# amcpherson/remixt

Hardware: AMD Instinct MI355X
Metric: EM iterations/sec (50k seg x 165 states) (higher is better)
Workload: dtype f64

## Files before the change

### include/remixt_amd.h

```cpp
#ifndef REMIXT_AMD_H
#define REMIXT_AMD_H

#include <stdint.h>

#ifdef __cplusplus
extern "C" {
#endif

#define RMX_OK 0
#define RMX_EVALUE 1
#define RMX_EASSERT 2
#define RMX_EDEVICE 3
#define RMX_EUNSUPPORTED 4
#define RMX_EARG 5

#define RMX_MAX_CLONES 4

typedef struct rmx_batch rmx_batch;

typedef struct rmx_problem {
    int32_t num_clones;
    int32_t num_segments;
    int32_t num_breakpoints;
    int32_t num_cn_states;
// ... 50 lines not shown
int rmx_info(rmx_batch *b, int32_t what, int64_t *out);
enum rmx_option_id {
    RMX_OPT_FB_KERNEL = 0,
    RMX_OPT_FB_NV,
    RMX_OPT_FB_BREAKEND_CODES,
    RMX_OPT_FUSE_SWEEPS,
    RMX_OPT_TWO_STREAMS,
    RMX_OPT_VITERBI_PLAIN,
    RMX_OPT_SEARCH_MODE,
    RMX_OPT_ELL_DENSE,
    RMX_OPT_STRIP,
    RMX_OPT_CELL_CACHE,
    RMX_OPT_SPARSE_TRIAL,
    RMX_OPT_FB_DEBUG,
    RMX_OPT_PAIRWISE_KERNEL,
    RMX_OPT_PACE_SWEEPS,
    RMX_OPT_FB_WG_BUDGET,
    RMX_OPT_TRIAL_KERNEL,
    RMX_OPT_GRAD_KERNEL,
    RMX_OPT_STREAM_POOL,
    RMX_OPT_VITERBI_CLUSTER,
    RMX_OPT_TRACEBACK,
    RMX_OPT_LT_CLASSES,
    RMX_OPT_COUNT
};
int rmx_set_default_option(int32_t option_id, int32_t value);
int rmx_set_option(rmx_batch *b, int32_t option_id, int32_t value);
int rmx_get_option(rmx_batch *b, int32_t option_id, int32_t *value);

int rmx_set_param(rmx_batch *b, int32_t r, int32_t param_id, double value);
int rmx_get_param(rmx_batch *b, int32_t r, int32_t param_id, double *value);
int rmx_set_transition_model(rmx_batch *b, int32_t model);
int rmx_set_array(rmx_batch *b, int32_t r, int32_t array_id, const void *host_src);
int rmx_get_array(rmx_batch *b, int32_t r, int32_t array_id, void *host_dst);
int rmx_fetch_indicators(rmx_batch *b, int32_t r0, int32_t r1, const double **total, const double **allele);
int rmx_calculate_log_transmat(rmx_batch *b, int32_t r, double *dst);
int rmx_weighted_search(const double *p, int64_t n, const double *u, int32_t k, int64_t *out, int64_t *positive);
int rmx_weighted_sample_round(const double *w, int64_t n, int64_t stride, double norm, const double *u, int32_t k,
                              int64_t *found, int32_t *nfound, int32_t cap, int64_t *positive);
int rmx_get_state_table(rmx_batch *b, int32_t which, int64_t *host_dst);

int rmx_update_framelogprob(rmx_batch *b, int32_t r0, int32_t r1);
int rmx_update_p_cn(rmx_batch *b, int32_t r0, int32_t r1);
int rmx_update_p_breakpoint(rmx_batch *b, int32_t r0, int32_t r1);
int rmx_update_p_outlier_total(rmx_batch *b, int32_t r0, int32_t r1);
int rmx_update_p_outlier_allele(rmx_batch *b, int32_t r0, int32_t r1);
// ... 69 lines not shown
```

### remixt_amd/bpmodel.py

```python
import ctypes as C

import numpy as np

from . import _lib

_dp = C.POINTER(C.c_double)
_ip = C.POINTER(C.c_int64)
_i32p = C.POINTER(C.c_int32)

RMX_EVALUE, RMX_EASSERT, RMX_EDEVICE, RMX_EUNSUPPORTED, RMX_EARG = 1, 2, 3, 4, 5

MAX_CLONES = 4
PARAM_IDS = {
    'negbin_r_0': 0, 'negbin_r_1': 1, 'negbin_hdel_mu': 2, 'negbin_hdel_r_0': 3, 'negbin_hdel_r_1': 4,
    'betabin_M_0': 5, 'betabin_M_1': 6, 'betabin_loh_p': 7, 'betabin_loh_M_0': 8, 'betabin_loh_M_1': 9,
    'prior_outlier_total': 10, 'prior_outlier_allele': 11, 'divergence_weight': 12, 'hmm_log_norm_const': 13,
}
ARRAY_IDS = {
    'h': 0, 'p_breakpoint': 1, 'p_allele_swap': 2, 'p_outlier_total': 3, 'p_outlier_allele': 4,
    'posterior_marginals': 5, 'framelogprob': 6, 'total_likelihood_mask': 7, 'allele_likelihood_mask': 8,
    'log_transmat': 9, 'cached_log_transmat': 10, 'joint_posterior_marginals': 11, 'state_sequence': 12,
}
_WRITABLE = {'h', 'p_breakpoint', 'p_allele_swap', 'p_outlier_total', 'p_outlier_allele', 'posterior_marginals',
             'total_likelihood_mask', 'allele_likelihood_mask'}
_STATE_TABLES = {'cn_states_total': 0, 'num_alleles_subclonal': 1, 'is_hdel': 2, 'is_loh': 3}


OPTION_IDS = dict((n, i) for i, n in enumerate((
    'fb_kernel', 'fb_nv', 'fb_breakend_codes', 'fuse_sweeps', 'two_streams', 'viterbi_plain', 'search_mode', 'ell_dense', 'strip',
    'cell_cache', 'sparse_trial', 'fb_debug', 'pairwise_kernel', 'pace_sweeps', 'fb_wg_budget', 'trial_kernel', 'grad_kernel', 'stream_pool', 'viterbi_cluster', 'traceback', 'lt_classes')))


def set_default_option(name, value):
    lib = _lib.load()
    rc = lib.rmx_set_default_option(OPTION_IDS[name], int(value))
    if rc:
        _raise(lib, rc)


def last_error_restarts():
    lib = _lib.load()
    n = lib.rmx_last_error_restarts(None, 0)
    if n <= 0:
        return []
    buf = (C.c_int32 * n)()
    n = min(n, lib.rmx_last_error_restarts(buf, n))
    return [int(buf[i]) for i in range(n)]


def _raise(lib, rc):
    msg = lib.rmx_last_error().decode()
    if rc == RMX_EVALUE:
        err = ValueError(msg)
# ... 803 lines not shown
```

### remixt_amd/csrc/rmx_api.hip

```cpp
#include <hip/hip_runtime.h>
#include <algorithm>
#include <cmath>
#include <limits>
#include <atomic>
#include <cstdio>
#include <cstring>
#include <functional>
#include <map>
#include <mutex>
#include <string>
#include <vector>
#include <chrono>
#include <cstdlib>
#include <condition_variable>
#include <memory>

#include "rmx_kernels.h"
#include "rmx_host.h"

static thread_local std::string g_err;
static thread_local std::vector<int32_t> g_err_restarts;
static int fail(int code, const std::string &msg) { g_err = msg; g_err_restarts.clear(); return code; }
static int fail_flagged(int code, const std::string &msg) { g_err = msg; return code; }
static inline long long now_ns() { return std::chrono::duration_cast<std::chrono::nanoseconds>(std::chrono::steady_clock::now().time_since_epoch()).count(); }
// ... 13 lines not shown
    "k_update_outlier_allele", "k_update_allele_swap", "k_brk_lut", "k_pairwise", "k_brk_update", "k_elbo_seg", "k_elbo_final",
    "k_ell_list", "k_ell_final", "k_ell_full", "k_viterbi", "k_backtrace", "other", "k_sample_cn", "k_posterior_summary", "k_region_prob", "k_region_counts", "k_call_prob", "k_region_moments"};

struct ProfRec { int id; hipEvent_t a, b; };

struct StreamPool { std::mutex mu; std::vector<hipStream_t> idle[2]; int created[2] = {0, 0}; };
static StreamPool g_stream_pool[16];
static int pool_acquire(int dev, int role, hipStream_t *out) {
    StreamPool &p = g_stream_pool[dev & 15];
    std::lock_guard<std::mutex> lk(p.mu);
    std::vector<hipStream_t> &idle = p.idle[role];
    if (!idle.empty()) { *out = idle.front(); idle.erase(idle.begin()); return RMX_OK; }
    if (hipStreamCreateWithFlags(out, hipStreamNonBlocking) != hipSuccess) return RMX_EDEVICE;
    p.created[role]++;
    return RMX_OK;
}
static void pool_release(int dev, int role, hipStream_t s) {
    hipStreamSynchronize(s);
    StreamPool &p = g_stream_pool[dev & 15];
    std::lock_guard<std::mutex> lk(p.mu);
    p.idle[role].push_back(s);
}

static int g_opt_default[RMX_OPT_COUNT] = {0, 0, 1, 1, 1, 0, 5, 0, 1, 1, 1, 0, 0, 0, 0, 0, 0, 1, 0, 0, 1};
static std::mutex g_opt_mu;

struct rmx_batch {
    hipEvent_t ev_pace = nullptr;
    int opt[RMX_OPT_COUNT];
    int device = 0;
    hipStream_t stream = nullptr;
    hipStream_t stream2 = nullptr;
    hipEvent_t ev_fb = nullptr, ev_brk = nullptr;
    bool own_stream = false, pooled_stream = false, pooled_stream2 = false;
    Dev d{};
    int R = 0;
    std::vector<int64_t> cn_classes;
    std::vector<int32_t> seg_class, brk_idx, brk_orient, tclass, brk_slot, be_n;
    std::vector<int64_t> brk_states, is_telomere;
    std::vector<std::pair<int, int>> tc_pairs;
    std::vector<double> Tsum;
    std::vector<RestartParams> rp;
    std::vector<char> tables_dirty, segc_dirty, ab_dirty;
    std::vector<double> segc_built;
    std::vector<char> sig_valid;
    std::vector<int> cache_stale;
    bool use_cache = false;
// ... 460 lines not shown
}
typedef void (*cells_kernel_t)(Dev, int);
template <int NS, int LTC> static cells_kernel_t cells_kernel_cached(int mode, int mask, int cache) {
    if (mode == 0) return cache == 2 ? k_cells<NS, 0, CM_ALL, 2, LTC> : k_cells<NS, 0, CM_ALL, 1, LTC>;
    if (mode == 1) return k_cells<NS, 1, CM_ALL, 2, LTC>;
    if (mode == 3) return k_cells<NS, 3, CM_ALL, 2, LTC>;
    if (cache == 2) return k_cells<NS, 2, 31, 2, LTC>;
    switch (mask) {
    case 1: return k_cells<NS, 2, 1, 1, LTC>; case 2: return k_cells<NS, 2, 2, 1, LTC>;
    case 3: return k_cells<NS, 2, 3, 1, LTC>; case 4: return k_cells<NS, 2, 4, 1, LTC>; case 8: return k_cells<NS, 2, 8, 1, LTC>;
    case 12: return k_cells<NS, 2, 12, 1, LTC>; case 15: return k_cells<NS, 2, 15, 1, LTC>; default: return k_cells<NS, 2, 31, 1, LTC>;
    }
}
template <int NS> static cells_kernel_t cells_kernel_ns(int mode, int mask, int cache, bool ltc) {
    if (cache) return ltc ? cells_kernel_cached<NS, 1>(mode, mask, cache) : cells_kernel_cached<NS, 0>(mode, mask, cache);
    if (mode == 0) return k_cells<NS, 0, CM_ALL, 0, 0>;
    if (mode == 1) return k_cells<NS, 1, CM_ALL, 0, 0>;
    switch (mask) {
    case 1: return k_cells<NS, 2, 1, 0, 0>; case 2: return k_cells<NS, 2, 2, 0, 0>;
    case 3: return k_cells<NS, 2, 3, 0, 0>; case 4: return k_cells<NS, 2, 4, 0, 0>; case 8: return k_cells<NS, 2, 8, 0, 0>;
    case 12: return k_cells<NS, 2, 12, 0, 0>; case 15: return k_cells<NS, 2, 15, 0, 0>; default: return k_cells<NS, 2, 31, 0, 0>;
    }
}
static bool use_strip(rmx_batch *b) { return b->d.S > 32 && b->d.S <= 384 && b->opt[RMX_OPT_STRIP]; }
static cells_kernel_t cells_kernel(rmx_batch *b, int mode, int mask, int cache) {
    const int ns = (b->d.S + 63) / 64;
    const bool ltc = cache != 0 && b->d.ltc != nullptr;
    switch (ns) { case 1: return cells_kernel_ns<1>(mode, mask, cache, ltc); case 2: return cells_kernel_ns<2>(mode, mask, cache, ltc);
                  case 3: return cells_kernel_ns<3>(mode, mask, cache, ltc); case 4: return cells_kernel_ns<4>(mode, mask, cache, ltc);
                  case 5: return cells_kernel_ns<5>(mode, mask, cache, ltc); default: return cells_kernel_ns<6>(mode, mask, cache, ltc); }
}
static dim3 ell_block(rmx_batch *b) { return dim3(std::min(256, ((b->d.S + 63) / 64) * 64)); }
static bool ell_sparse_ok(rmx_batch *b, int n, const int32_t *restarts) {
    if (!b->d.sig_cnt || b->opt[RMX_OPT_ELL_DENSE]) return false;
    for (int i = 0; i < n; i++) if (!b->sig_valid[restarts[i]]) return false;
    return true;
}
static dim3 strip_grid(rmx_batch *b, int nr) { return dim3((b->d.N + 4 * STRIP_RPW - 1) / (4 * STRIP_RPW), nr); }
static int cover_mask(int m) {
    if (m & 16) return 31;
    if ((m & 3) && (m & 12)) return 15;
    if ((m & 3) == 3) return 3;
    if (m & 1) return 1;
    if (m & 2) return 2;
    if ((m & 12) == 12) return 12;
    if (m & 4) return 4;
    if (m & 8) return 8;
    return 0;
}

// ... 695 lines not shown
    return RMX_OK;
}

int rmx_get_state_table(rmx_batch *b, int32_t which, int64_t *dst) { BIND(b);
    const Dev &d = b->d;
    const int S = d.S, M = d.M;
    for (int n = 0; n < d.N; n++) {
        const int64_t *t = b->cn_classes.data() + (size_t)b->seg_class[n] * S * M * 2;
        for (int s = 0; s < S; s++) {
            if (which == 0) { for (int m = 0; m < M; m++) dst[((size_t)n * S + s) * M + m] = t[(s * M + m) * 2] + t[(s * M + m) * 2 + 1]; continue; }
            bool hdel = true, loh = false; int nsub = 0;
            for (int m = 0; m < M; m++) if (t[(s * M + m) * 2] || t[(s * M + m) * 2 + 1]) hdel = false;
            for (int a = 0; a < 2; a++) {
                int64_t sum = 0; for (int m = 0; m < M; m++) sum += t[(s * M + m) * 2 + a];
                if (sum == 0) loh = true;
                if (M > 1) { int64_t lo = t[(s * M + 1) * 2 + a], hi = lo; for (int m = 2; m < M; m++) { lo = std::min(lo, t[(s * M + m) * 2 + a]); hi = std::max(hi, t[(s * M + m) * 2 + a]); } if (hi != lo) nsub++; }
            }
            dst[(size_t)n * S + s] = which == 1 ? nsub : (which == 2 ? (hdel ? 1 : 0) : (loh ? 1 : 0));
        }
    }
    return RMX_OK;
}

static int do_framelogprob(rmx_batch *b, int r0, int r1) {
    int rc = ensure_tables(b, r0, r1);
    if (rc) return rc;
    ProfScope ps(b, KID_FRAMELOGPROB);
    if (use_strip(b)) {
        int r = r0;
        while (r < r1) {
            const bool cur = b->use_cache && b->cache_stale[r] == 0;
            int e = r;
            while (e < r1 && (b->use_cache && b->cache_stale[e] == 0) == cur) e++;
            hipLaunchKernelGGL(cells_kernel(b, 0, CM_ALL, cur ? 2 : (b->use_cache ? 1 : 0)), strip_grid(b, e - r), dim3(256), 0, b->stream, b->d, r);
            if (b->use_cache) for (int i = r; i < e; i++) b->cache_stale[i] = 0;
            r = e;
        }
    }
    else hipLaunchKernelGGL(k_framelogprob, row_grid(b, r1 - r0), dim3(256), 0, b->stream, b->d, r0, b->G);
    HIPCHK(hipGetLastError());
    return RMX_OK;
}
static inline int fb_wg_budget(const rmx_batch *b) { return b->opt[RMX_OPT_FB_WG_BUDGET] > 0 ? b->opt[RMX_OPT_FB_WG_BUDGET] : b->num_cus; }
static void (*fbm_kernel_for(int KB))(FbmArgs) {
    switch (KB) { case 8: return k_fbm<8>; case 16: return k_fbm<16>; case 28: return k_fbm<28>; case 36: return k_fbm<36>; case 42: return k_fbm<42>; case 44: return k_fbm<44>; }
    return nullptr;
}
static int fb_items_for(rmx_batch *b, int r0, int r1, int pin, const double (&cost)[5], rmx_batch::FbItems **out) {
    if ((pin == 1 || pin == 2 || pin == 4) && cost[pin] == 0.) pin = 4;
    auto key = std::make_tuple(r0, r1, pin * 4096 + fb_wg_budget(b));
    auto it = b->fb_items.find(key);
    if (it != b->fb_items.end()) { *out = &it->second; return RMX_OK; }
    std::vector<int> shapes;
    for (int nv : {4, 2, 1}) if (cost[nv] > 0.) shapes.push_back(nv);
    const int nc = (int)b->h_list_fast.size();
    auto units = [&](int nv) { return (r1 - 1) / nv - r0 / nv + 1; };
    std::vector<int> nv_of(nc, 4);
// ... 10 lines not shown
                if (!pick) ok = false; else { nv_of[c] = pick; wg += 2L * units(pick); }
            }
            if (ok && wg <= fb_wg_budget(b)) break;
            std::fill(nv_of.begin(), nv_of.end(), 4);
        }
    }
    std::vector<int> order(nc);
    for (int c = 0; c < nc; c++) order[c] = c;
    std::stable_sort(order.begin(), order.end(), [&](int x, int y) { return b->h_chain_len[b->h_list_fast[x]] * cost[nv_of[x]] > b->h_chain_len[b->h_list_fast[y]] * cost[nv_of[y]]; });
    std::vector<int4> items;
    rmx_batch::FbItems f;
    for (int c : order) {
        const int nv = nv_of[c];
        f.nv_min = std::min(f.nv_min, nv); f.nv_max = std::max(f.nv_max, nv);
        for (int u = r0 / nv; u <= (r1 - 1) / nv; u++) for (int dir = 0; dir < 2; dir++) items.push_back(make_int4(b->h_list_fast[c], u * nv, nv, dir));
    }
    f.n = (int)items.size();
    int rc = dalloc(b, &f.dev, items.size());
    if (rc) return rc;
    HIPCHK(hipMemcpy(f.dev, items.data(), items.size() * sizeof(int4), hipMemcpyHostToDevice));
    *out = &(b->fb_items[key] = f);
    return RMX_OK;
}
static int p_cn_front(rmx_batch *b, int r0, int r1, bool skip_frame, bool snapshot_done = false) {
    int rc = skip_frame ? ensure_tables(b, r0, r1) : do_framelogprob(b, r0, r1);
    if (rc) return rc;
    if (!snapshot_done && (rc = launch_brk_lut(b, r0, r1, b->d.pd_lt, b->d.pe_lt))) return rc;
    {
        ProfScope ps(b, KID_FB);
        const Dev &d = b->d;
        FbArgs a;
        a.S = d.S; a.SP = d.SP; a.M = d.M; a.D = d.D; a.C = d.C; a.N = d.N; a.NBE = d.NBE; a.cn_max = d.cn_max;
        a.r0 = r0; a.pen = d.pen;
        a.chain_start = d.chain_start; a.chain_end = d.chain_end; a.tclass = d.tclass; a.brk_slot = d.brk_slot;
        a.chain_tc = d.chain_tc; a.chain_cls = d.chain_cls; a.be_cls = d.be_cls; a.amat_lds = 0; a.pad_ = 0;
        a.fe = d.fe; a.Wf = d.Wf; a.Wb = d.Wb; a.pe_lt = d.pe_lt; a.af = d.af; a.ab = d.ab; a.tot = d.tot;
        a.fa = d.fa; a.fb = d.fb; a.mrow = d.mrow; a.err = d.err; a.dbg = b->d_dbg;
        bool fast = false;
        bool done_fast = false;
        if (b->fbv_rpt > 0 && b->n_fast > 0 && d.M <= 3 && (d.NBE == 0 || (d.pe2x_lt != nullptr && b->max_adist < 64 && b->opt[RMX_OPT_FB_BREAKEND_CODES])) &&
            b->opt[RMX_OPT_FB_KERNEL] != 3) {
            int KB = 0;
            for (int v : {8, 16, 28, 36, 42, 44}) if (4 * v >= d.S) { KB = v; break; }
            const int NCT = (d.S + 14) / 15;
            rmx_batch::FbItems *items = nullptr;
            static const double fbm_cost[5] = {0., 1500., 2110., 0., 2845.};
            if ((rc = fb_items_for(b, r0, r1, b->opt[RMX_OPT_FB_NV], fbm_cost, &items))) return rc;
            FbmArgs m;
// ... 119 lines not shown
        if (!fast) { b->last_fb_kernel = 0; b->last_fb_nv = b->last_fb_nv_max = 1; }
        const int ngen = fast ? b->n_generic : d.NC;
        if (ngen > 0) {
            a.amat_lds = 0; a.P = b->fbG.P; a.BLK = b->fbG.BLK; a.SPAD = b->fbG.SPAD; a.chain_list = fast ? d.chain_list_generic : d.chain_list_all;
            hipLaunchKernelGGL(fb_kernel_for(0), dim3(ngen, r1 - r0, 2), dim3(b->fbG.NT), b->fbG_lds, b->stream, a);
        }
        HIPCHK(hipGetLastError());
    }
    for (int r = r0; r < r1; r++) b->lt_model[r] = b->d.tmodel;
    for (int r = r0; r < r1; r++) { if (!b->lt_valid[r]) { b->lt_valid[r] = 1; int one = 1; HIPCHK(hipMemcpyAsync(b->d_lt_valid + r, &one, 4, hipMemcpyHostToDevice, b->stream)); } }
    return RMX_OK;
}
static int p_cn_marginals(rmx_batch *b, int r0, int r1, bool fuse_next) {
    {
        ProfScope ps(b, KID_MARGINALS);
        if (use_strip(b)) hipLaunchKernelGGL(cells_kernel(b, fuse_next ? 3 : 1, CM_ALL, b->use_cache ? 2 : 0), strip_grid(b, r1 - r0), dim3(256), 0, b->stream, b->d, r0);
        else hipLaunchKernelGGL(k_marginals<true>, row_grid(b, r1 - r0), dim3(256), 0, b->stream, b->d, r0, b->G);
        HIPCHK(hipGetLastError());
    }
    if (fuse_next && use_strip(b)) std::swap(b->d.fe, b->d.fe_alt);
    for (int r = r0; r < r1; r++) { b->ab_dirty[r] = 0; b->comp_dirty[r] = 0; b->comp_base[r] = 0; b->logz_dirty[r] = 1; b->sig_valid[r] = (!fuse_next && use_strip(b) && b->d.sig_cnt) ? 1 : 0; b->sig_epoch[r]++; }
    return RMX_OK;
}
static int do_update_p_cn(rmx_batch *b, int r0, int r1, bool skip_frame = false, bool fuse_next = false) {
    int rc;
    if ((rc = p_cn_front(b, r0, r1, skip_frame)) || (rc = launch_pairwise_breakends(b, r0, r1, 0))) return rc;
    return p_cn_marginals(b, r0, r1, fuse_next);
}
static int do_update_p_breakpoint(rmx_batch *b, int r0, int r1, bool snapshot = false) {
    const Dev &d = b->d;
    if (d.K > 0 && d.NBE > 0) {
        ProfScope ps(b, KID_BRK_UPDATE);
        hipLaunchKernelGGL(k_brk_update_lut, dim3(d.K, r1 - r0), dim3(128), (size_t)d.B * 16, b->stream, b->d, r0, b->d.pd_cached,
                           snapshot ? b->d.pd_lt : (double *)nullptr, b->d.pe_lt, b->d.pe2_lt, b->pe2p);
        HIPCHK(hipGetLastError());
    } else {
        if (d.K > 0) {
            ProfScope ps(b, KID_BRK_UPDATE);
            hipLaunchKernelGGL(k_brk_update, dim3(d.K, r1 - r0), dim3(128), (size_t)d.B * 16, b->stream, b->d, r0);
            HIPCHK(hipGetLastError());
        }
        int rc = launch_brk_lut(b, r0, r1, b->d.pd_cached, nullptr);
        if (rc) return rc;
        if (snapshot && (rc = launch_brk_lut(b, r0, r1, b->d.pd_lt, b->d.pe_lt))) return rc;
    }
    const double pti = plain_T_mean_sum(b);
    for (int r = r0; r < r1; r++) { b->plain_T_init[r] = pti; b->cached_model[r] = b->d.tmodel; }
    return RMX_OK;
}
// ... 7 lines not shown
    HIPCHK(hipGetLastError());
    return RMX_OK;
}

int rmx_update_framelogprob(rmx_batch *b, int32_t r0, int32_t r1) { BIND(b); RANGE_CHECK(); int rc = do_framelogprob(b, r0, r1); return rc ? rc : check_errors(b, r0, r1); }
int rmx_update_p_cn(rmx_batch *b, int32_t r0, int32_t r1) { BIND(b); RANGE_CHECK(); int rc = do_update_p_cn(b, r0, r1); return rc ? rc : check_errors(b, r0, r1); }
int rmx_update_p_breakpoint(rmx_batch *b, int32_t r0, int32_t r1) { BIND(b); RANGE_CHECK(); int rc = do_update_p_breakpoint(b, r0, r1); return rc ? rc : check_errors(b, r0, r1); }
int rmx_update_p_outlier_total(rmx_batch *b, int32_t r0, int32_t r1) { BIND(b); RANGE_CHECK(); int rc = do_indicator(b, r0, r1, 0); return rc ? rc : check_errors(b, r0, r1); }
int rmx_update_p_outlier_allele(rmx_batch *b, int32_t r0, int32_t r1) { BIND(b); RANGE_CHECK(); int rc = do_indicator(b, r0, r1, 1); return rc ? rc : check_errors(b, r0, r1); }
int rmx_update_p_allele_swap(rmx_batch *b, int32_t r0, int32_t r1) { BIND(b); RANGE_CHECK(); int rc = do_indicator(b, r0, r1, 2); return rc ? rc : check_errors(b, r0, r1); }

int rmx_variational_update(rmx_batch *b, int32_t r0, int32_t r1, int32_t iters) { BIND(b);
    RANGE_CHECK();
    const bool fusable = use_strip(b) && b->use_cache && b->opt[RMX_OPT_FUSE_SWEEPS];
    const bool two_streams = use_strip(b) && b->d.NBE > 0 && b->opt[RMX_OPT_TWO_STREAMS];
    if (two_streams && !b->stream2) {
        if (b->opt[RMX_OPT_STREAM_POOL]) { if (pool_acquire(b->device, 1, &b->stream2) != RMX_OK) return fail(RMX_EDEVICE, "hipStreamCreate failed"); b->pooled_stream2 = true; }
        else HIPCHK(hipStreamCreateWithFlags(&b->stream2, hipStreamNonBlocking));
        HIPCHK(hipEventCreateWithFlags(&b->ev_fb, hipEventDisableTiming));
        HIPCHK(hipEventCreateWithFlags(&b->ev_brk, hipEventDisableTiming));
    }
    bool snapshot_done = false;
    const bool paced = b->opt[RMX_OPT_PACE_SWEEPS] != 0;
    if (paced && !b->ev_pace) HIPCHK(hipEventCreateWithFlags(&b->ev_pace, hipEventDisableTiming));
    for (int it = 0; it < iters; it++) {
        int rc;
        if (paced && it > 0) HIPCHK(hipEventSynchronize(b->ev_pace));
        const bool fused_in = fusable && it > 0, fuse_out = fusable && it + 1 < iters;
        if (!fused_in && (rc = do_indicator(b, r0, r1, 2))) return rc;
        if (two_streams) {
            if ((rc = p_cn_front(b, r0, r1, fused_in, snapshot_done))) return rc;
            if (paced) HIPCHK(hipEventRecord(b->ev_pace, b->stream));
            hipStream_t main_stream = b->stream;
            HIPCHK(hipEventRecord(b->ev_fb, main_stream));
            HIPCHK(hipStreamWaitEvent(b->stream2, b->ev_fb, 0));
            b->stream = b->stream2;
            rc = launch_pairwise_breakends(b, r0, r1, 0);
            snapshot_done = it + 1 < iters;
            if (!rc) rc = do_update_p_breakpoint(b, r0, r1, snapshot_done);
            b->stream = main_stream;
            if (rc) return rc;
            HIPCHK(hipEventRecord(b->ev_brk, b->stream2));
            if ((rc = p_cn_marginals(b, r0, r1, fuse_out))) return rc;
            HIPCHK(hipStreamWaitEvent(main_stream, b->ev_brk, 0));
        } else {
            if ((rc = do_update_p_cn(b, r0, r1, fused_in, fuse_out)) || (rc = do_update_p_breakpoint(b, r0, r1))) return rc;
            if (paced) HIPCHK(hipEventRecord(b->ev_pace, b->stream));
        }
        if (!fuse_out && ((rc = do_indicator(b, r0, r1, 0)) || (rc = do_indicator(b, r0, r1, 1)))) return rc;
    }
    return check_errors(b, r0, r1);
}

static int elbo_parts(rmx_batch *b, int r0, int r1, bool exact_parts, double *out4 ) {
    int rc = ensure_ab(b, r0, r1);
    if (rc) return rc;
    const int nr = r1 - r0;
    const double *full_plain = nullptr;
    if (exact_parts) {
        for (int r = r0; r < r1; r++) if (!b->lt_valid[r]) exact_parts = false;
    }
    std::vector<double> plain_host;
    double *d_fp = nullptr;
    if (exact_parts && !b->plain_list.empty()) {
        const int np = (int)b->plain_list.size();
        if (!b->d_plain_list) { if ((rc = dalloc(b, &b->d_plain_list, np)) || (rc = dalloc(b, &b->d_plain_jt, (size_t)b->R * np))) return rc;
            HIPCHK(hipMemcpy(b->d_plain_list, b->plain_list.data(), (size_t)np * 4, hipMemcpyHostToDevice)); }
        { ProfScope ps(b, KID_PAIRWISE);
          for (int r = r0; r < r1; r++)
// ... 1348 lines not shown
```

### remixt_amd/csrc/rmx_device.h

```cpp
#pragma once
#include <hip/hip_runtime.h>
#include <stdint.h>
#include "../../include/remixt_amd.h"

#define RMX_ERR_NAN_LL 1u
#define RMX_ERR_BAD_P 2u
#define RMX_ERR_TOTAL_DEPTH 4u
#define RMX_ERR_LOH_P 8u
#define RMX_ERR_NAN_F 16u
#define RMX_ERR_NAN_AB 32u
#define RMX_ERR_NAN_POST 64u
#define RMX_ERR_DIGAMMA 128u
#define RMX_ERR_NAN_GRAD 256u

#define ST_HDEL_NB 1u
#define ST_LOH_M 2u
#define ST_E_TD 4u
#define ST_E_LOH 8u
#define ST_E_BADP 16u
#define ST_GZ_ALLELE 32u

struct RestartParams {
    double h[RMX_MAX_CLONES];
    double p[RMX_P_COUNT];
    double logr[2];
};

struct Dev {
    int N, S, SP, M, K, B, C, D, cn_max, NC, NBE, TC, nc, tmodel, R, pad0;
    double pen;
    const double *l, *x, *y, *logl;
    const uint8_t *mask_t, *mask_a;
    const int32_t *seg_class;
    const int32_t *tclass;
    const int32_t *brk_slot;
    const int32_t *brk_idx, *brk_orient;
    const int32_t *be_n;
    const int32_t *chain_be;
    const int32_t *be_cls;
    const int32_t *chain_tc;
    const int32_t *chain_cls;
    const int32_t *chain_list_fast, *chain_list_generic, *chain_list_all;
    const int32_t *chain_start, *chain_end;
    const uint8_t *chain_end_flag;
    const int8_t *cn;
    const int8_t *tot;
    const uint8_t *sflags;
    const int32_t *brk_states;
    const int32_t *bk_ptr, *bk_slots;
    const double *Tval, *Wf, *Wb;
    const int8_t *af, *ab;
    const uint16_t *pcode;
// ... 371 lines not shown
```

### remixt_amd/csrc/rmx_kernels.h

```cpp
#pragma once
#include "rmx_device.h"
#include "rmx_host.h"
#define SEGL 32
#define SEG_PER_BLOCK (256 / SEGL)
#define TRIAL_SEGL 16
#define RMX_CLUSTER_SPINS (1u << 22)
#define FBK_WKN 128
#define NM_MAX_SAMPLE 1024
#define TRIAL_SEG_PER_BLOCK (256 / TRIAL_SEGL)


__device__ __forceinline__ void state_tables_body(const Dev &d, int cls, int r, const RestartParams &rp) {
    __shared__ unsigned agg_sh;
    if (threadIdx.x == 0) agg_sh = 0u;
    __syncthreads();
    unsigned agg = 0u;
    for (int s = threadIdx.x; s < d.S; s += blockDim.x) {
        const int8_t *cn = d.cn + ((size_t)cls * d.S + s) * d.M * 2;
        const int8_t *tot = d.tot + ((size_t)cls * d.S + s) * d.M;
        double minor = 0., total = 0.;
        for (int m = 0; m < d.M; m++) {
            minor += rp.h[m] * (double)cn[m * 2 + 0];
            total += rp.h[m] * (double)tot[m];
        }
// ... 1713 lines not shown
                    }
                }
            }
            __builtin_amdgcn_wave_barrier();
        };
        if (MODE == 0) {
            const double qt0 = d.qt[rn * 2], qt1 = d.qt[rn * 2 + 1], qa0 = d.qa[rn * 2], qa1 = d.qa[rn * 2 + 1];
            const double qs0 = d.qs[rn * 2], qs1 = d.qs[rn * 2 + 1];
            double fv[NS];
            double vmax = -INFINITY;
            lt_rows_to_lds();
#pragma unroll
            for (int k = 0; k < NS; k++) {
                const int s = lane + 64 * k;
                fv[k] = -INFINITY;
                if (s < S) {
                    double LT[2], LA[4];
                    cell(sc, st[k], (size_t)n * d.SP + s, k, LT, LA);
                    double f = 0.;
                    f += qt0 * LT[0]; f += qt1 * LT[1];
                    f += qa0 * qs0 * LA[0]; f += qa0 * qs1 * LA[1]; f += qa1 * qs0 * LA[2]; f += qa1 * qs1 * LA[3];
                    f += -1.0 * (CACHE == 2 ? nsub_of(cls, s) : st[k].nsub) * sc.l * divw;
                    if (f != f) err |= RMX_ERR_NAN_F;
                    d.f[ro + s] = f;
                    fv[k] = f;
                    vmax = fmax(vmax, f);
                }
                __builtin_amdgcn_sched_barrier(0);
            }
            vmax = group_max(vmax, 64);
            if (lane == 0) d.fmax[rn] = vmax;
#pragma unroll
            for (int k = 0; k < NS; k++) { const int s = lane + 64 * k; if (s < d.SP) d.fe[ro + s] = s < S ? exp_fast(fv[k] - vmax) : 0.; }
        } else {
            constexpr bool M1 = MODE == 1 || MODE == 3;
            constexpr int LAOFF = LTC ? 0 : 2;
            constexpr int NSTASH = MODE != 3 ? 0 : LTC ? (NS <= 3 ? 4 : (NS == 4 ? 3 : 2)) : (NS <= 3 ? 6 : (NS <= 6 ? 3 : 0));
            constexpr bool STASH = NSTASH > 0;
            __shared__ double lsm[STASH ? 4 : 1][STASH ? NS * NSTASH * 64 : 1];
            double pv[NS];
            double sum = 0.;
            if (M1) {
#pragma unroll
                for (int k = 0; k < NS; k++) {
                    const int s = lane + 64 * k;
                    pv[k] = PREFETCH ? pfa[PREFETCH ? k : 0] * pfb[PREFETCH ? k : 0] : (s < S ? d.fa[ro + s] * d.fb[ro + s] : 0.);
                    sum += pv[k];
// ... 116 lines not shown
                            if (LTC) lt_gather(k, LT);
                            else {
#pragma unroll
                                for (int q_ = 0; q_ < 2; q_++) LT[q_] = q_ < NSTASH ? lsm[wave][(k * NSTASH + q_) * 64 + lane] : lcr[q_ * plane + off_];
                            }
#pragma unroll
                            for (int q_ = 0; q_ < 4; q_++) LA[q_] = LAOFF + q_ < NSTASH ? lsm[wave][(k * NSTASH + LAOFF + q_) * 64 + lane] : lar[q_ * plane + off_];
                        } else cell(sc, st[k], (size_t)n * d.SP + s, k, LT, LA);
                        double f = 0.;
                        f += qt0 * LT[0]; f += qt1 * LT[1];
                        f += qa0 * qs0 * LA[0]; f += qa0 * qs1 * LA[1]; f += qa1 * qs0 * LA[2]; f += qa1 * qs1 * LA[3];
                        f += -1.0 * nsub_of(cls, s) * sc.l * divw;
                        if (f != f) err |= RMX_ERR_NAN_F;
                        fv[k] = f;
                        vmax = fmax(vmax, f);
                    }
                }
                vmax = group_max(vmax, 64);
                if (lane == 0) d.fmax[rn] = vmax;
#pragma unroll
                for (int k = 0; k < NS; k++) { const int s = lane + 64 * k; if (s < d.SP) d.fe_alt[ro + s] = s < S ? exp_fast(fv[k] - vmax) : 0.; }
            }
        }
    }
    if (err) atomicOr(&d.err[r], err);
}

template <int MASK>
__global__ __launch_bounds__(256) void k_trial_sparse(Dev d, int r0) {
    const int r = r0 + blockIdx.y;
    const int n = blockIdx.x * TRIAL_SEG_PER_BLOCK + (threadIdx.x / TRIAL_SEGL), j = threadIdx.x & (TRIAL_SEGL - 1);
    if (n >= d.N) return;
    const RestartParams &rp = d.rp[r];
    SegCtx sc; load_seg(d, r, n, sc);
    const int cls = d.seg_class[n];
    const size_t rn = (size_t)r * d.N + n;
    const double *post = d.post + rn * d.SP;
    const int cnt = d.sig_cnt[rn];
    unsigned err = 0;
    double a0 = 0., a1 = 0., b0 = 0., b1 = 0., b2 = 0., b3 = 0.;
    auto one = [&](int s) {
        StateRegs st; load_state_regs(d, r, cls, s, st);
        double LT[2], LA[4];
        cell_ll_regs<MASK>(rp, sc, st, LT, LA, err);
        const double ps = post[s];
        a0 += ps * LT[0]; a1 += ps * LT[1];
// ... 3382 lines not shown
```

Measured before the change: 461.0.

## Add software-pipelined cached cells kernel and skip redundant frame log-prob stores

Adds a new k_cells_pipe kernel for cached frame and marginal passes with 65–192 states. Each wave prefetches the next segment's cached likelihood planes, forward/backward values and scalars into registers while it computes the current one, staging them through LDS. The kernel uses a launch-bounds occupancy hint. Separately, in strip mode the frame pass no longer writes the full f array, since the marginal pass recomputes it. The costs are higher register pressure from the prefetch buffers and more kernel template instantiations; whether dropping f is safe depends on every consumer getting it elsewhere.

```diff
diff --git a/include/remixt_amd.h b/include/remixt_amd.h
--- a/include/remixt_amd.h
+++ b/include/remixt_amd.h
@@ -96,6 +96,7 @@
     RMX_OPT_VITERBI_CLUSTER,
     RMX_OPT_TRACEBACK,
     RMX_OPT_LT_CLASSES,
+    RMX_OPT_CELLS_PIPELINE,
     RMX_OPT_COUNT
 };
 int rmx_set_default_option(int32_t option_id, int32_t value);
diff --git a/remixt_amd/bpmodel.py b/remixt_amd/bpmodel.py
--- a/remixt_amd/bpmodel.py
+++ b/remixt_amd/bpmodel.py
@@ -28,7 +28,7 @@
 
 OPTION_IDS = dict((n, i) for i, n in enumerate((
     'fb_kernel', 'fb_nv', 'fb_breakend_codes', 'fuse_sweeps', 'two_streams', 'viterbi_plain', 'search_mode', 'ell_dense', 'strip',
-    'cell_cache', 'sparse_trial', 'fb_debug', 'pairwise_kernel', 'pace_sweeps', 'fb_wg_budget', 'trial_kernel', 'grad_kernel', 'stream_pool', 'viterbi_cluster', 'traceback', 'lt_classes')))
+    'cell_cache', 'sparse_trial', 'fb_debug', 'pairwise_kernel', 'pace_sweeps', 'fb_wg_budget', 'trial_kernel', 'grad_kernel', 'stream_pool', 'viterbi_cluster', 'traceback', 'lt_classes', 'cells_pipeline')))
 
 
 def set_default_option(name, value):
diff --git a/remixt_amd/csrc/rmx_api.hip b/remixt_amd/csrc/rmx_api.hip
--- a/remixt_amd/csrc/rmx_api.hip
+++ b/remixt_amd/csrc/rmx_api.hip
@@ -59,7 +59,7 @@
     p.idle[role].push_back(s);
 }
 
-static int g_opt_default[RMX_OPT_COUNT] = {0, 0, 1, 1, 1, 0, 5, 0, 1, 1, 1, 0, 0, 0, 0, 0, 0, 1, 0, 0, 1};
+static int g_opt_default[RMX_OPT_COUNT] = {0, 0, 1, 1, 1, 0, 5, 0, 1, 1, 1, 0, 0, 0, 0, 0, 0, 1, 0, 0, 1, 1};
 static std::mutex g_opt_mu;
 
 struct rmx_batch {
@@ -566,10 +566,18 @@
     case 12: return k_cells<NS, 2, 12, 0, 0>; case 15: return k_cells<NS, 2, 15, 0, 0>; default: return k_cells<NS, 2, 31, 0, 0>;
     }
 }
+template <int NS> static cells_kernel_t cells_kernel_pipe(int mode, bool ltc) {
+    if (mode == 0) return ltc ? k_cells_pipe<NS, 0, 1> : k_cells_pipe<NS, 0, 0>;
+    if (mode == 1) return ltc ? k_cells_pipe<NS, 1, 1> : k_cells_pipe<NS, 1, 0>;
+    return ltc ? k_cells_pipe<NS, 3, 1> : k_cells_pipe<NS, 3, 0>;
+}
 static bool use_strip(rmx_batch *b) { return b->d.S > 32 && b->d.S <= 384 && b->opt[RMX_OPT_STRIP]; }
 static cells_kernel_t cells_kernel(rmx_batch *b, int mode, int mask, int cache) {
     const int ns = (b->d.S + 63) / 64;
     const bool ltc = cache != 0 && b->d.ltc != nullptr;
+    static_assert(CELLS_PIPE_MINNS == 2 && CELLS_PIPE_MAXNS == 3, "one case per state count below");
+    if (cache == 2 && mode != 2 && ns >= CELLS_PIPE_MINNS && ns <= CELLS_PIPE_MAXNS && b->opt[RMX_OPT_CELLS_PIPELINE])
+        return ns == 2 ? cells_kernel_pipe<2>(mode, ltc) : cells_kernel_pipe<3>(mode, ltc);
     switch (ns) { case 1: return cells_kernel_ns<1>(mode, mask, cache, ltc); case 2: return cells_kernel_ns<2>(mode, mask, cache, ltc);
                   case 3: return cells_kernel_ns<3>(mode, mask, cache, ltc); case 4: return cells_kernel_ns<4>(mode, mask, cache, ltc);
                   case 5: return cells_kernel_ns<5>(mode, mask, cache, ltc); default: return cells_kernel_ns<6>(mode, mask, cache, ltc); }
@@ -1311,17 +1319,19 @@
     return RMX_OK;
 }
 
-static int do_framelogprob(rmx_batch *b, int r0, int r1) {
+static int do_framelogprob(rmx_batch *b, int r0, int r1, bool store_f = true) {
     int rc = ensure_tables(b, r0, r1);
     if (rc) return rc;
     ProfScope ps(b, KID_FRAMELOGPROB);
     if (use_strip(b)) {
+        Dev dv = b->d;
+        dv.skip_f = store_f ? 0 : 1;
         int r = r0;
         while (r < r1) {
             const bool cur = b->use_cache && b->cache_stale[r] == 0;
             int e = r;
             while (e < r1 && (b->use_cache && b->cache_stale[e] == 0) == cur) e++;
-            hipLaunchKernelGGL(cells_kernel(b, 0, CM_ALL, cur ? 2 : (b->use_cache ? 1 : 0)), strip_grid(b, e - r), dim3(256), 0, b->stream, b->d, r);
+            hipLaunchKernelGGL(cells_kernel(b, 0, CM_ALL, cur ? 2 : (b->use_cache ? 1 : 0)), strip_grid(b, e - r), dim3(256), 0, b->stream, dv, r);
             if (b->use_cache) for (int i = r; i < e; i++) b->cache_stale[i] = 0;
             r = e;
         }
@@ -1378,8 +1388,8 @@
     *out = &(b->fb_items[key] = f);
     return RMX_OK;
 }
-static int p_cn_front(rmx_batch *b, int r0, int r1, bool skip_frame, bool snapshot_done = false) {
-    int rc = skip_frame ? ensure_tables(b, r0, r1) : do_framelogprob(b, r0, r1);
+static int p_cn_front(rmx_batch *b, int r0, int r1, bool skip_frame, bool snapshot_done = false, bool store_f = true) {
+    int rc = skip_frame ? ensure_tables(b, r0, r1) : do_framelogprob(b, r0, r1, store_f);
     if (rc) return rc;
     if (!snapshot_done && (rc = launch_brk_lut(b, r0, r1, b->d.pd_lt, b->d.pe_lt))) return rc;
     {
@@ -1545,9 +1555,9 @@
     for (int r = r0; r < r1; r++) { b->ab_dirty[r] = 0; b->comp_dirty[r] = 0; b->comp_base[r] = 0; b->logz_dirty[r] = 1; b->sig_valid[r] = (!fuse_next && use_strip(b) && b->d.sig_cnt) ? 1 : 0; b->sig_epoch[r]++; }
     return RMX_OK;
 }
-static int do_update_p_cn(rmx_batch *b, int r0, int r1, bool skip_frame = false, bool fuse_next = false) {
+static int do_update_p_cn(rmx_batch *b, int r0, int r1, bool skip_frame = false, bool fuse_next = false, bool store_f = true) {
     int rc;
-    if ((rc = p_cn_front(b, r0, r1, skip_frame)) || (rc = launch_pairwise_breakends(b, r0, r1, 0))) return rc;
+    if ((rc = p_cn_front(b, r0, r1, skip_frame, false, store_f)) || (rc = launch_pairwise_breakends(b, r0, r1, 0))) return rc;
     return p_cn_marginals(b, r0, r1, fuse_next);
 }
 static int do_update_p_breakpoint(rmx_batch *b, int r0, int r1, bool snapshot = false) {
@@ -1601,6 +1611,7 @@
     }
     bool snapshot_done = false;
     const bool paced = b->opt[RMX_OPT_PACE_SWEEPS] != 0;
+    const bool store_f = !use_strip(b);
     if (paced && !b->ev_pace) HIPCHK(hipEventCreateWithFlags(&b->ev_pace, hipEventDisableTiming));
     for (int it = 0; it < iters; it++) {
         int rc;
@@ -1608,7 +1619,7 @@
         const bool fused_in = fusable && it > 0, fuse_out = fusable && it + 1 < iters;
         if (!fused_in && (rc = do_indicator(b, r0, r1, 2))) return rc;
         if (two_streams) {
-            if ((rc = p_cn_front(b, r0, r1, fused_in, snapshot_done))) return rc;
+            if ((rc = p_cn_front(b, r0, r1, fused_in, snapshot_done, store_f))) return rc;
             if (paced) HIPCHK(hipEventRecord(b->ev_pace, b->stream));
             hipStream_t main_stream = b->stream;
             HIPCHK(hipEventRecord(b->ev_fb, main_stream));
@@ -1623,7 +1634,7 @@
             if ((rc = p_cn_marginals(b, r0, r1, fuse_out))) return rc;
             HIPCHK(hipStreamWaitEvent(main_stream, b->ev_brk, 0));
         } else {
-            if ((rc = do_update_p_cn(b, r0, r1, fused_in, fuse_out)) || (rc = do_update_p_breakpoint(b, r0, r1))) return rc;
+            if ((rc = do_update_p_cn(b, r0, r1, fused_in, fuse_out, store_f)) || (rc = do_update_p_breakpoint(b, r0, r1))) return rc;
             if (paced) HIPCHK(hipEventRecord(b->ev_pace, b->stream));
         }
         if (!fuse_out && ((rc = do_indicator(b, r0, r1, 0)) || (rc = do_indicator(b, r0, r1, 1)))) return rc;
diff --git a/remixt_amd/csrc/rmx_device.h b/remixt_amd/csrc/rmx_device.h
--- a/remixt_amd/csrc/rmx_device.h
+++ b/remixt_amd/csrc/rmx_device.h
@@ -27,7 +27,8 @@
 };
 
 struct Dev {
-    int N, S, SP, M, K, B, C, D, cn_max, NC, NBE, TC, nc, tmodel, R, pad0;
+    int N, S, SP, M, K, B, C, D, cn_max, NC, NBE, TC, nc, tmodel, R;
+    int skip_f;
     double pen;
     const double *l, *x, *y, *logl;
     const uint8_t *mask_t, *mask_a;
diff --git a/remixt_amd/csrc/rmx_kernels.h b/remixt_amd/csrc/rmx_kernels.h
--- a/remixt_amd/csrc/rmx_kernels.h
+++ b/remixt_amd/csrc/rmx_kernels.h
@@ -1759,7 +1759,7 @@
                     f += qa0 * qs0 * LA[0]; f += qa0 * qs1 * LA[1]; f += qa1 * qs0 * LA[2]; f += qa1 * qs1 * LA[3];
                     f += -1.0 * (CACHE == 2 ? nsub_of(cls, s) : st[k].nsub) * sc.l * divw;
                     if (f != f) err |= RMX_ERR_NAN_F;
-                    d.f[ro + s] = f;
+                    if (!d.skip_f) d.f[ro + s] = f;
                     fv[k] = f;
                     vmax = fmax(vmax, f);
                 }
@@ -1922,6 +1922,253 @@
                 for (int k = 0; k < NS; k++) { const int s = lane + 64 * k; if (s < d.SP) d.fe_alt[ro + s] = s < S ? exp_fast(fv[k] - vmax) : 0.; }
             }
         }
+    }
+    if (err) atomicOr(&d.err[r], err);
+}
+
+#define CELLS_PIPE_MINNS 2
+#define CELLS_PIPE_MAXNS 3
+#define CELLS_PIPE_WAVES 3
+template <int NS, int MODE, int LTC>
+__global__ __launch_bounds__(256, CELLS_PIPE_WAVES) void k_cells_pipe(Dev d, int r0) {
+    static_assert(NS >= CELLS_PIPE_MINNS && NS <= CELLS_PIPE_MAXNS && (MODE == 0 || MODE == 1 || MODE == 3), "cached frame / marginal passes, 65 .. 192 states");
+    constexpr bool M1 = MODE != 0;
+    constexpr int NP = LTC ? 4 : 6, LAOFF = LTC ? 0 : 2;
+    constexpr int NSV = MODE == 1 ? 9 : 7;
+    const int r = r0 + blockIdx.y;
+    const int lane = threadIdx.x & 63;
+    const int wave = __builtin_amdgcn_readfirstlane((int)(threadIdx.x >> 6));
+    const int nbeg = (blockIdx.x * 4 + wave) * STRIP_RPW;
+    if (nbeg >= d.N) return;
+    const int nend = min(d.N, nbeg + STRIP_RPW);
+    const RestartParams &rp = d.rp[r];
+    const int S = d.S;
+    unsigned err = 0;
+    const double divw = rp.p[RMX_P_DIVERGENCE_WEIGHT];
+    const size_t plane = (size_t)d.N * d.SP;
+    const double *lcr = d.lc + (size_t)r * NP * plane;
+    const size_t lplane = LTC ? (size_t)d.N * d.NTP : 0;
+    const double *ltr = LTC ? d.ltc + (size_t)r * 2 * lplane : nullptr;
+    __shared__ double ltl[LTC ? 4 : 1][LTC ? 256 : 1];
+    __shared__ double lsm[4][NS * NP * 64];
+    int cur_cls = -1;
+    unsigned ci = 0u, nsb = 0u;
+    auto lane_of = [&](double v, int l_) { return __hiloint2double(__builtin_amdgcn_readlane(__double2hiint(v), l_), __builtin_amdgcn_readlane(__double2loint(v), l_)); };
+    auto nsub_k = [&](int k) { return (double)((nsb >> (2 * k)) & 3u); };
+    auto cell = [&](int k, double LT[2], double LA[4]) {
+        if (LTC) { const unsigned c_ = (ci >> (8 * k)) & 0xffu; LT[0] = ltl[wave][c_]; LT[1] = ltl[wave][128 + c_]; }
+        else { LT[0] = lsm[wave][(k * NP) * 64 + lane]; LT[1] = lsm[wave][(k * NP + 1) * 64 + lane]; }
+#pragma unroll
+        for (int q_ = 0; q_ < 4; q_++) LA[q_] = lsm[wave][(k * NP + LAOFF + q_) * 64 + lane];
+    };
+    double lp_prior[4] = {0., 0., 0., 0.};
+    if (MODE == 3) {
+        const double pt_ = rp.p[RMX_P_PRIOR_OUTLIER_TOTAL], pa_ = rp.p[RMX_P_PRIOR_OUTLIER_ALLELE];
+        lp_prior[0] = log_prior(1. - pt_); lp_prior[1] = log_prior(pt_); lp_prior[2] = log_prior(1. - pa_); lp_prior[3] = log_prior(pa_);
+    }
+    auto uni = [](size_t v_) {
+        return ((size_t)(unsigned)__builtin_amdgcn_readfirstlane((int)(v_ >> 32)) << 32) | (unsigned)__builtin_amdgcn_readfirstlane((int)v_);
+    };
+    auto at = [](const double *base, unsigned off) { return *(const double *)((const char *)base + off); };
+    unsigned os[NS], oc[2];
+#pragma unroll
+    for (int k = 0; k < NS; k++) os[k] = 8u * (unsigned)min(lane + 64 * k, S - 1);
+    oc[0] = LTC ? 8u * (unsigned)min(lane, d.NT - 1) : 0u; oc[1] = LTC ? 8u * (unsigned)min(lane + 64, d.NT - 1) : 0u;
+    double nfa[M1 ? NS : 1], nfb[M1 ? NS : 1], npl[NS][NP], nlt[LTC ? 4 : 1] = {}, nsv = 0.;
+    int ncls = 0, ncef = 0;
+    auto request = [&](int n) {
+        const size_t rn = (size_t)r * d.N + n, ro = rn * d.SP, co = (size_t)n * d.SP;
+        ncls = d.seg_class[n];
+        if (MODE == 1) ncef = d.chain_end_flag[n];
+        const double *sp_ = lane < 2 ? d.qt + rn * 2 + lane : lane < 4 ? d.qa + rn * 2 + (lane - 2) : lane < 6 ? d.qs + rn * 2 + (lane - 4)
+                          : lane == 6 ? d.l + n : lane == 7 ? d.fmax + rn : d.mrow + rn;
+        nsv = *sp_;
+        if (LTC) {
+            const double *lt0_ = ltr + uni((size_t)n * d.NTP), *lt1_ = ltr + uni(lplane + (size_t)n * d.NTP);
+            nlt[0] = at(lt0_, oc[0]); nlt[LTC ? 1 : 0] = at(lt1_, oc[0]);
+            if (d.NT > 64) { nlt[LTC ? 2 : 0] = at(lt0_, oc[1]); nlt[LTC ? 3 : 0] = at(lt1_, oc[1]); }
+        }
+        if (M1) {
+            const size_t ro_ = uni(ro);
+            const double *fa_ = d.fa + ro_, *fb_ = d.fb + ro_;
+#pragma unroll
+            for (int k = 0; k < NS; k++) { nfa[M1 ? k : 0] = at(fa_, os[k]); nfb[M1 ? k : 0] = at(fb_, os[k]); }
+        }
+#pragma unroll
+        for (int q_ = 0; q_ < NP; q_++) {
+            const double *pl_ = lcr + uni(q_ * plane + co);
+#pragma unroll
+            for (int k = 0; k < NS; k++) npl[k][q_] = at(pl_, os[k]);
+        }
+    };
+    request(nbeg);
+    for (int n = nbeg; n < nend; n++) {
+        const size_t rn = (size_t)r * d.N + n;
+        const size_t ro = rn * d.SP;
+        const int cls = __builtin_amdgcn_readfirstlane(ncls);
+        const int cef = MODE == 1 ? __builtin_amdgcn_readfirstlane(ncef) : 0;
+        const double q0 = MODE != 3 ? lane_of(nsv, 0) : 0., q1 = MODE != 3 ? lane_of(nsv, 1) : 0., q2 = MODE != 3 ? lane_of(nsv, 2) : 0., q3 = MODE != 3 ? lane_of(nsv, 3) : 0.;
+        const double q4 = lane_of(nsv, 4), q5 = lane_of(nsv, 5), sl = lane_of(nsv, 6);
+        const double fmx = MODE == 1 ? lane_of(nsv, 7) : 0., mrw = MODE == 1 ? lane_of(nsv, 8) : 0.;
+        if (LTC) {
+            if (lane < d.NT) { ltl[wave][lane] = nlt[0]; ltl[wave][128 + lane] = nlt[LTC ? 1 : 0]; }
+            if (d.NT > 64 && lane + 64 < d.NT) { ltl[wave][64 + lane] = nlt[LTC ? 2 : 0]; ltl[wave][192 + lane] = nlt[LTC ? 3 : 0]; }
+        }
+        double pv[NS];
+        double sum = 0.;
+#pragma unroll
+        for (int k = 0; k < NS; k++) {
+            if (M1) { const bool in_ = lane + 64 * k < S; const double a_ = in_ ? nfa[M1 ? k : 0] : 0., b_ = in_ ? nfb[M1 ? k : 0] : 0.; pv[k] = __dmul_rn(a_, b_); sum = __fma_rn(a_, b_, sum); }
+#pragma unroll
+            for (int q_ = 0; q_ < NP; q_++) lsm[wave][(k * NP + q_) * 64 + lane] = npl[k][q_];
+        }
+        __builtin_amdgcn_wave_barrier();
+        if (cls != cur_cls) {
+            ci = 0u; nsb = 0u;
+#pragma unroll
+            for (int k = 0; k < NS; k++) {
+                const int s = lane + 64 * k;
+                const size_t si = (size_t)cls * S + (s < S ? s : S - 1);
+                if (LTC) ci |= (unsigned)d.ltcls[si] << (8 * k);
+                nsb |= ((unsigned)(d.sflags[si] >> 2) & 3u) << (2 * k);
+            }
+            cur_cls = cls;
+        }
+        if (n + 1 < nend) request(n + 1);
+        if (MODE == 0) {
+            double fv[NS];
+            double vmax = -INFINITY;
+#pragma unroll
+            for (int k = 0; k < NS; k++) {
+                const int s = lane + 64 * k;
+                fv[k] = -INFINITY;
+                if (s < S) {
+                    double LT[2], LA[4];
+                    cell(k, LT, LA);
+                    double f = 0.;
+                    f += q0 * LT[0]; f += q1 * LT[1];
+                    f += q2 * q4 * LA[0]; f += q2 * q5 * LA[1]; f += q3 * q4 * LA[2]; f += q3 * q5 * LA[3];
+                    f += -1.0 * nsub_k(k) * sl * divw;
+                    if (f != f) err |= RMX_ERR_NAN_F;
+                    if (!d.skip_f) d.f[ro + s] = f;
+                    fv[k] = f;
+                    vmax = fmax(vmax, f);
+                }
+            }
+            vmax = group_max(vmax, 64);
+            if (lane == 0) d.fmax[rn] = vmax;
+#pragma unroll
+            for (int k = 0; k < NS; k++) { const int s = lane + 64 * k; if (s < d.SP) d.fe[ro + s] = s < S ? exp_fast(fv[k] - vmax) : 0.; }
+        } else {
+            sum = group_sum(sum, 64);
+            if (!(sum > 0.) || sum != sum || sum == INFINITY) err |= RMX_ERR_NAN_POST;
+            double s2 = 0.;
+#pragma unroll
+            for (int k = 0; k < NS; k++) { pv[k] = pv[k] / sum; s2 += pv[k]; }
+            s2 = group_sum(s2, 64);
+#pragma unroll
+            for (int k = 0; k < NS; k++) { const int s = lane + 64 * k; pv[k] = pv[k] / s2; if (MODE != 3 && s < S) d.post[ro + s] = pv[k]; }
+            if (MODE == 1 && d.sig_cnt) {
+                int base_ = 0;
+#pragma unroll
+                for (int k = 0; k < NS; k++) {
+                    const int s = lane + 64 * k;
+                    const bool sg_ = s < S && pv[k] >= RMX_POST_EPS;
+                    const unsigned long long bal_ = __ballot(sg_);
+                    const int pos_ = base_ + __popcll(bal_ & ((1ull << lane) - 1ull));
+                    if (sg_ && pos_ < RMX_SIGK) d.sig_idx[rn * RMX_SIGK + pos_] = (uint16_t)s;
+                    base_ += __popcll(bal_);
+                }
+                if (lane == 0) d.sig_cnt[rn] = base_ <= RMX_SIGK ? (uint8_t)base_ : (uint8_t)255;
+            }
+            double a0 = 0., a1 = 0., b0 = 0., b1 = 0., b2 = 0., b3 = 0., pf = 0., pp = 0.;
+#pragma unroll
+            for (int k = 0; k < NS; k++) {
+                const int s = lane + 64 * k;
+                if (s < S) {
+                    double LT[2], LA[4];
+                    cell(k, LT, LA);
+                    const double ps = pv[k];
+                    a0 += ps * LT[0]; a1 += ps * LT[1];
+                    b0 += ps * LA[0]; b1 += ps * LA[1]; b2 += ps * LA[2]; b3 += ps * LA[3];
+                    if (MODE == 1) {
+                        double f = 0.;
+                        f += q0 * LT[0]; f += q1 * LT[1];
+                        f += q2 * q4 * LA[0]; f += q2 * q5 * LA[1]; f += q3 * q4 * LA[2]; f += q3 * q5 * LA[3];
+                        f += -1.0 * nsub_k(k) * sl * divw;
+                        d.f[ro + s] = f;
+                        pf += ps * f;
+                        pp += ps * (-1.0 * nsub_k(k) * sl * divw);
+                    }
+                }
+            }
+            a0 = group_sum(a0, 64); if (lane == 0) d.A[rn * 2] = a0;
+            a1 = group_sum(a1, 64); if (lane == 0) d.A[rn * 2 + 1] = a1;
+            b0 = group_sum(b0, 64); b1 = group_sum(b1, 64); if (lane == 0) { d.Bv[rn * 4] = b0; d.Bv[rn * 4 + 1] = b1; }
+            b2 = group_sum(b2, 64); b3 = group_sum(b3, 64); if (lane == 0) { d.Bv[rn * 4 + 2] = b2; d.Bv[rn * 4 + 3] = b3; }
+            if (MODE == 1) {
+                pf = group_sum(pf, 64); pp = group_sum(pp, 64);
+                if (lane == 0) { d.rowPF[rn] = pf; d.rowPP[rn] = pp; }
+                if (lane == 0) d.rowZ[rn] = fmx + (cef ? log(sum) : log(mrw));
+            }
+            if (MODE == 3) {
+                auto b0_ = [](double v) { return __hiloint2double(__builtin_amdgcn_readfirstlane(__double2hiint(v)), __builtin_amdgcn_readfirstlane(__double2loint(v))); };
+                a0 = b0_(a0); a1 = b0_(a1); b0 = b0_(b0); b1 = b0_(b1); b2 = b0_(b2); b3 = b0_(b3);
+                double lpt0 = lp_prior[0], lpt1 = lp_prior[1];
+                lpt0 += a0; lpt1 += a1;
+                const double qs0o = q4, qs1o = q5;
+                double lpa0, lpa1;
+                outlier_allele_logits(lp_prior[2], lp_prior[3], qs0o, qs1o, b0, b1, b2, b3, lpa0, lpa1);
+                const double vmt = lpt0 > lpt1 ? lpt0 : lpt1, vma = lpa0 > lpa1 ? lpa0 : lpa1;
+                const double lp_l = lane == 0 ? lpt0 : (lane == 1 ? lpt1 : (lane == 2 ? lpa0 : lpa1));
+                const double vm_l = lane < 2 ? vmt : vma;
+                const double ex = exp_fast(lp_l - vm_l);
+                double pst = 0.; pst += lane_of(ex, 0); pst += lane_of(ex, 1);
+                double psa = 0.; psa += lane_of(ex, 2); psa += lane_of(ex, 3);
+                const double lg = fast_log_pos(lane < 2 ? pst : psa);
+                const double norm_l = lg + vm_l;
+                const double y_l = exp_fast(lp_l - norm_l);
+                double qt0 = lane_of(y_l, 0), qt1 = lane_of(y_l, 1), qa0 = lane_of(y_l, 2), qa1 = lane_of(y_l, 3);
+                { const double st_ = qt0 + qt1; qt0 /= st_; qt1 /= st_; const double sa_ = qa0 + qa1; qa0 /= sa_; qa1 /= sa_; }
+                double lps0, lps1;
+                allele_swap_logits(qa0, qa1, b0, b1, b2, b3, lps0, lps1);
+                const double vms = lps0 > lps1 ? lps0 : lps1;
+                const double lps_l = (lane & 1) ? lps1 : lps0;
+                const double exs = exp_fast(lps_l - vms);
+                double pss = 0.; pss += lane_of(exs, 0); pss += lane_of(exs, 1);
+                const double norms = fast_log_pos(pss) + vms;
+                const double ys_l = exp_fast(lps_l - norms);
+                double qs0 = lane_of(ys_l, 0), qs1 = lane_of(ys_l, 1);
+                { const double ss_ = qs0 + qs1; qs0 /= ss_; qs1 /= ss_; }
+                if (lane == 0) {
+                    d.qt[rn * 2] = qt0; d.qt[rn * 2 + 1] = qt1; d.qa[rn * 2] = qa0; d.qa[rn * 2 + 1] = qa1;
+                    d.qs[rn * 2] = qs0; d.qs[rn * 2 + 1] = qs1;
+                }
+                double fv[NS];
+                double vmax = -INFINITY;
+#pragma unroll
+                for (int k = 0; k < NS; k++) {
+                    const int s = lane + 64 * k;
+                    fv[k] = -INFINITY;
+                    if (s < S) {
+                        double LT[2], LA[4];
+                        cell(k, LT, LA);
+                        double f = 0.;
+                        f += qt0 * LT[0]; f += qt1 * LT[1];
+                        f += qa0 * qs0 * LA[0]; f += qa0 * qs1 * LA[1]; f += qa1 * qs0 * LA[2]; f += qa1 * qs1 * LA[3];
+                        f += -1.0 * nsub_k(k) * sl * divw;
+                        if (f != f) err |= RMX_ERR_NAN_F;
+                        fv[k] = f;
+                        vmax = fmax(vmax, f);
+                    }
+                }
+                vmax = group_max(vmax, 64);
+                if (lane == 0) d.fmax[rn] = vmax;
+#pragma unroll
+                for (int k = 0; k < NS; k++) { const int s = lane + 64 * k; if (s < d.SP) d.fe_alt[ro + s] = s < S ? exp_fast(fv[k] - vmax) : 0.; }
+            }
+        }
+        __builtin_amdgcn_wave_barrier();
     }
     if (err) atomicOr(&d.err[r], err);
 }
```

After: 476.5 (median of 6 runs). +3.4%, better.
